# neeharperi/FutureDet

Hardware: AMD Instinct MI355X
Metric: sweeps/sec end-to-end (300k pts, 10-sweep voxel) (higher is better)
Workload: dtype f32

## Files before the change

### futuredet_amd/csrc/fd_spconv_c32.hip

```cpp
#include "fd_spconv_chunk.h"

namespace {

namespace sk = fd::skeleton;
typedef float f32x16 __attribute__((ext_vector_type(16)));
typedef unsigned u32x4 __attribute__((ext_vector_type(4)));
constexpr int TM = 128, COUT = 32, TS = 4, WR = 1;
constexpr sk::Layout L = sk::layout(TM, COUT, TS, 32);
static_assert(((sk::kMaxTaps + TS - 1) / TS) * (TM / WR / 32) <= L.item_slot, "item list slot");

template <int CIN, int DEPTH>
__global__ void __launch_bounds__(256) spconv_f32_c32(const float *__restrict__ in, const float4 *__restrict__ wp, const float *__restrict__ bias,
                                                      const float *__restrict__ residual, int relu, const int *__restrict__ nbr, int64_t nbr_stride,
                                                      int K, int n_out, const int *__restrict__ n_out_dev, float *__restrict__ out, unsigned in_bytes,
                                                      const int *__restrict__ ranges, int rows_per_range) {
    constexpr int NCH = CIN / 8;
    constexpr int kPad = sk::pad_entry(TM);
    extern __shared__ __attribute__((aligned(16))) unsigned char smem[];
    int *s_list = reinterpret_cast<int *>(smem + L.list);
    unsigned short *s_items = reinterpret_cast<unsigned short *>(smem + L.items);
    unsigned char *s_cnt = smem + L.cnt;
    int *s_pad = reinterpret_cast<int *>(smem + L.pad);
    float *s_acc = reinterpret_cast<float *>(smem + L.acc);

    const int tid = threadIdx.x, lane = tid & 63, wave = __builtin_amdgcn_readfirstlane(tid >> 6);
    int r_begin, r_end, n_chunks, chunk_rows;
    sk::resolve_range(n_out, n_out_dev, ranges, rows_per_range, r_begin, r_end);
    if (r_begin >= r_end) return;
    sk::cut_chunks<TM>(r_begin, r_end, n_chunks, chunk_rows);
    int pre[sk::kSliceRegs<TM>];
    sk::fetch_slice<TM>(pre, nbr, nbr_stride, K, r_begin);

    const int ln = lane & 31, lh = lane >> 5;
    const int ts = wave, wr = 0;
    unsigned char *acc_bytes = reinterpret_cast<unsigned char *>(s_acc + ts * L.acc_copy);
    const __amdgpu_buffer_rsrc_t rsrc = __builtin_amdgcn_make_buffer_rsrc(const_cast<float *>(in), 0, (int)in_bytes, 0x00020000);
    unsigned short *items = s_items + wave * L.item_slot;

    for (int chunk = 0; chunk < n_chunks; ++chunk) {
        int row0, n_rows;
        if (!sk::chunk_span(r_begin, r_end, chunk_rows, chunk, row0, n_rows)) break;
        sk::stage_chunk<TM, COUT, TS, 32>(pre, s_list, s_pad, s_acc, bias, residual, K, row0, n_rows);
        __syncthreads();
        sk::compact_taps<TM, WR>(s_list, s_cnt, K);
        __syncthreads();
        if (chunk + 1 < n_chunks) sk::fetch_slice<TM>(pre, nbr, nbr_stride, K, row0 + chunk_rows);
        const int n_items = sk::build_items<TS, 32>(s_cnt, items, K, ts, wr);

        int k_r[DEPTH], row_r[DEPTH];
        u32x4 a_r[DEPTH][NCH];
        auto stage_a0 = [&](int it) -> int { return sk::stage_a0(items, n_items, it); };
        auto stage_a1 = [&](int it, int code_v, int &kk, int &e) { sk::stage_a1<TM, WR, 32>(s_list, s_pad, n_items, wr, ln, it, code_v, kk, e); };
        auto gather_offset = [&](int e) -> unsigned { return sk::entry_row_bytes<CIN>(e) + (unsigned)(lh * 16); };
        auto gather_step = [&](unsigned voff, int c) { return __builtin_amdgcn_raw_buffer_load_b128(rsrc, voff + c * 32, 0, 0); };
        float4 b[NCH];
        auto load_b = [&](int k) {
            const float4 *wk = wp + (int64_t)k * NCH * 64 + lane;
#pragma unroll
            for (int c = 0; c < NCH; ++c) b[c] = wk[c * 64];
        };
        int k_s, e_s, code_s;
#pragma unroll
        for (int d = 0; d < DEPTH - 1; ++d) {
            stage_a1(d, stage_a0(d), k_s, e_s);
            const unsigned vo = gather_offset(e_s);
#pragma unroll
            for (int c = 0; c < NCH; ++c) a_r[d][c] = gather_step(vo, c);
            k_r[d] = k_s;
            row_r[d] = e_s;
        }
        k_r[DEPTH - 1] = -1;
        row_r[DEPTH - 1] = kPad;
        stage_a1(DEPTH - 1, stage_a0(DEPTH - 1), k_s, e_s);
        code_s = stage_a0(DEPTH);
        if (n_items > 0) load_b(k_r[0]);

        for (int i0 = 0; i0 < n_items; i0 += DEPTH) {
#pragma unroll
            for (int d = 0; d < DEPTH; ++d) {
                const unsigned arow = sk::entry_local_row(row_r[d]);
                unsigned aoff[4];
#pragma unroll
                for (int q = 0; q < 4; ++q) aoff[q] = sk::acc_slot_bytes<COUT>(arow, (unsigned)(2 * q + lh));
                f32x16 acc;
#pragma unroll
                for (int q = 0; q < 4; ++q) {
                    const float4 v = *reinterpret_cast<const float4 *>(acc_bytes + aoff[q]);
                    acc[4 * q + 0] = v.x; acc[4 * q + 1] = v.y; acc[4 * q + 2] = v.z; acc[4 * q + 3] = v.w;
                }
                const int dn = (d + DEPTH - 1) % DEPTH;
                {
                    const int it = i0 + d + DEPTH - 1;
                    const unsigned vo = gather_offset(e_s);
                    k_r[dn] = k_s;
                    row_r[dn] = e_s;
#pragma unroll
                    for (int c = 0; c < NCH; ++c) a_r[dn][c] = gather_step(vo, c);
                    stage_a1(it + 1, code_s, k_s, e_s);
                    code_s = stage_a0(it + 2);
                }
                const int knext = k_r[(d + 1) % DEPTH];
                const bool reload = knext >= 0 && knext != k_r[d];
                __builtin_amdgcn_sched_barrier(0);
#pragma unroll
                for (int c = 0; c < NCH; ++c) {
                    const float4 av = __builtin_bit_cast(float4, a_r[d][c]);
                    acc = __builtin_amdgcn_mfma_f32_32x32x2f32(b[c].x, av.x, acc, 0, 0, 0);
                    acc = __builtin_amdgcn_mfma_f32_32x32x2f32(b[c].y, av.y, acc, 0, 0, 0);
                    acc = __builtin_amdgcn_mfma_f32_32x32x2f32(b[c].z, av.z, acc, 0, 0, 0);
                    acc = __builtin_amdgcn_mfma_f32_32x32x2f32(b[c].w, av.w, acc, 0, 0, 0);
                    if (reload) b[c] = (wp + (int64_t)knext * NCH * 64 + lane)[c * 64];
                }
#pragma unroll
                for (int q = 0; q < 4; ++q)
                    *reinterpret_cast<float4 *>(acc_bytes + aoff[q]) = make_float4(acc[4 * q + 0], acc[4 * q + 1], acc[4 * q + 2], acc[4 * q + 3]);
                __builtin_amdgcn_sched_barrier(0);
            }
        }
        __syncthreads();
        sk::epilogue<TM, COUT, TS>(s_acc, bias, residual, relu, out, row0, n_rows);
        __syncthreads();
    }
}

template <int CIN, int DEPTH>
int launch_c32(const fd::SpconvCall &c) {
    const unsigned in_bytes = (unsigned)(c.n_in * CIN * 4);
    int n_ranges = c.n_ranges, rows_per = 0;
    if (!c.ranges) sk::equal_rows_split(c.n_out, TM, c.n_out_dev != nullptr, n_ranges, rows_per);
    static std::atomic<uint64_t> lds_set{0};
    if (!fd::ensure_dynamic_lds(reinterpret_cast<const void *>(spconv_f32_c32<CIN, DEPTH>), (size_t)L.bytes, lds_set)) return 0;
    const void *wp = (const char *)c.wpacked + fd::spconv_weight_layout(c).c32.offset;
    hipLaunchKernelGGL((spconv_f32_c32<CIN, DEPTH>), dim3((unsigned)n_ranges), dim3(256), (size_t)L.bytes, c.stream, (const float *)c.in, (const float4 *)wp,
                       c.bias, (const float *)c.residual, c.relu, c.nbr, c.nbr_stride, c.K, c.n_out, c.n_out_dev, (float *)c.out, in_bytes, c.ranges, rows_per);
    return 1;
}

}

namespace fd {
int spconv_f32_c32_dispatch(const SpconvCall &c) {
    if (c.cout != 32 || c.cin != 32) return 0;
    if (!sk::entries_fit(c.n_in, c.cin)) return 0;
    return launch_c32<32, 3>(c);
}
}
```

Measured before the change: 282.1.

## Keep per-wave tap weights resident in registers and cut pipeline depth

```diff
diff --git a/futuredet_amd/csrc/fd_spconv_c32.hip b/futuredet_amd/csrc/fd_spconv_c32.hip
--- a/futuredet_amd/csrc/fd_spconv_c32.hip
+++ b/futuredet_amd/csrc/fd_spconv_c32.hip
@@ -6,11 +6,12 @@
 typedef float f32x16 __attribute__((ext_vector_type(16)));
 typedef unsigned u32x4 __attribute__((ext_vector_type(4)));
 constexpr int TM = 128, COUT = 32, TS = 4, WR = 1;
+constexpr int NSET = (sk::kMaxTaps + TS - 1) / TS;
 constexpr sk::Layout L = sk::layout(TM, COUT, TS, 32);
 static_assert(((sk::kMaxTaps + TS - 1) / TS) * (TM / WR / 32) <= L.item_slot, "item list slot");
 
 template <int CIN, int DEPTH>
-__global__ void __launch_bounds__(256) spconv_f32_c32(const float *__restrict__ in, const float4 *__restrict__ wp, const float *__restrict__ bias,
+__global__ void __launch_bounds__(256) __attribute__((amdgpu_waves_per_eu(2, 2))) spconv_f32_c32(const float *__restrict__ in, const float4 *__restrict__ wp, const float *__restrict__ bias,
                                                       const float *__restrict__ residual, int relu, const int *__restrict__ nbr, int64_t nbr_stride,
                                                       int K, int n_out, const int *__restrict__ n_out_dev, float *__restrict__ out, unsigned in_bytes,
                                                       const int *__restrict__ ranges, int rows_per_range) {
@@ -28,11 +29,31 @@
     sk::resolve_range(n_out, n_out_dev, ranges, rows_per_range, r_begin, r_end);
     if (r_begin >= r_end) return;
     sk::cut_chunks<TM>(r_begin, r_end, n_chunks, chunk_rows);
-    int pre[sk::kSliceRegs<TM>];
-    sk::fetch_slice<TM>(pre, nbr, nbr_stride, K, r_begin);
-
     const int ln = lane & 31, lh = lane >> 5;
     const int ts = wave, wr = 0;
+    float4 w[NSET][NCH];
+#pragma unroll
+    for (int s = 0; s < NSET; ++s) {
+        const int k = ts + TS * s < K ? ts + TS * s : K - 1;
+        const float4 *wk = wp + (int64_t)k * NCH * 64 + lane;
+#pragma unroll
+        for (int c = 0; c < NCH; ++c) w[s][c] = wk[c * 64];
+    }
+    int pre[sk::kSliceRegs<TM>];
+    static_assert(256 % TM == 0 && 64 % (256 / TM) == 0, "a wave stays inside one tap");
+    auto fetch_slice = [&](int row0) {
+        int64_t o = (int64_t)row0 + tid % TM;
+        o = o < nbr_stride ? o : nbr_stride - 1;
+        const int *col = nbr + o;
+#pragma unroll
+        for (int i = 0; i < sk::kSliceRegs<TM>; ++i) {
+            int k = wave / (TM / 64) + i * (256 / TM);
+            k = k < K ? k : K - 1;
+            pre[i] = col[(int64_t)k * nbr_stride];
+        }
+    };
+    fetch_slice(r_begin);
+
     unsigned char *acc_bytes = reinterpret_cast<unsigned char *>(s_acc + ts * L.acc_copy);
     const __amdgpu_buffer_rsrc_t rsrc = __builtin_amdgcn_make_buffer_rsrc(const_cast<float *>(in), 0, (int)in_bytes, 0x00020000);
     unsigned short *items = s_items + wave * L.item_slot;
@@ -44,7 +65,7 @@
         __syncthreads();
         sk::compact_taps<TM, WR>(s_list, s_cnt, K);
         __syncthreads();
-        if (chunk + 1 < n_chunks) sk::fetch_slice<TM>(pre, nbr, nbr_stride, K, row0 + chunk_rows);
+        if (chunk + 1 < n_chunks) fetch_slice(row0 + chunk_rows);
         const int n_items = sk::build_items<TS, 32>(s_cnt, items, K, ts, wr);
 
         int k_r[DEPTH], row_r[DEPTH];
@@ -53,12 +74,6 @@
         auto stage_a1 = [&](int it, int code_v, int &kk, int &e) { sk::stage_a1<TM, WR, 32>(s_list, s_pad, n_items, wr, ln, it, code_v, kk, e); };
         auto gather_offset = [&](int e) -> unsigned { return sk::entry_row_bytes<CIN>(e) + (unsigned)(lh * 16); };
         auto gather_step = [&](unsigned voff, int c) { return __builtin_amdgcn_raw_buffer_load_b128(rsrc, voff + c * 32, 0, 0); };
-        float4 b[NCH];
-        auto load_b = [&](int k) {
-            const float4 *wk = wp + (int64_t)k * NCH * 64 + lane;
-#pragma unroll
-            for (int c = 0; c < NCH; ++c) b[c] = wk[c * 64];
-        };
         int k_s, e_s, code_s;
 #pragma unroll
         for (int d = 0; d < DEPTH - 1; ++d) {
@@ -68,12 +83,12 @@
             for (int c = 0; c < NCH; ++c) a_r[d][c] = gather_step(vo, c);
             k_r[d] = k_s;
             row_r[d] = e_s;
+            __builtin_amdgcn_sched_barrier(0);
         }
         k_r[DEPTH - 1] = -1;
         row_r[DEPTH - 1] = kPad;
         stage_a1(DEPTH - 1, stage_a0(DEPTH - 1), k_s, e_s);
         code_s = stage_a0(DEPTH);
-        if (n_items > 0) load_b(k_r[0]);
 
         for (int i0 = 0; i0 < n_items; i0 += DEPTH) {
 #pragma unroll
@@ -99,17 +114,20 @@
                     stage_a1(it + 1, code_s, k_s, e_s);
                     code_s = stage_a0(it + 2);
                 }
-                const int knext = k_r[(d + 1) % DEPTH];
-                const bool reload = knext >= 0 && knext != k_r[d];
                 __builtin_amdgcn_sched_barrier(0);
+                const int slot = k_r[d] >> 2;
+                static_assert(TS == 4 && NSET == 7, "tap -> weight set");
 #pragma unroll
-                for (int c = 0; c < NCH; ++c) {
-                    const float4 av = __builtin_bit_cast(float4, a_r[d][c]);
-                    acc = __builtin_amdgcn_mfma_f32_32x32x2f32(b[c].x, av.x, acc, 0, 0, 0);
-                    acc = __builtin_amdgcn_mfma_f32_32x32x2f32(b[c].y, av.y, acc, 0, 0, 0);
-                    acc = __builtin_amdgcn_mfma_f32_32x32x2f32(b[c].z, av.z, acc, 0, 0, 0);
-                    acc = __builtin_amdgcn_mfma_f32_32x32x2f32(b[c].w, av.w, acc, 0, 0, 0);
-                    if (reload) b[c] = (wp + (int64_t)knext * NCH * 64 + lane)[c * 64];
+                for (int s = 0; s < NSET; ++s) {
+                    if (slot != s) continue;
+#pragma unroll
+                    for (int c = 0; c < NCH; ++c) {
+                        const float4 av = __builtin_bit_cast(float4, a_r[d][c]);
+                        acc = __builtin_amdgcn_mfma_f32_32x32x2f32(w[s][c].x, av.x, acc, 0, 0, 0);
+                        acc = __builtin_amdgcn_mfma_f32_32x32x2f32(w[s][c].y, av.y, acc, 0, 0, 0);
+                        acc = __builtin_amdgcn_mfma_f32_32x32x2f32(w[s][c].z, av.z, acc, 0, 0, 0);
+                        acc = __builtin_amdgcn_mfma_f32_32x32x2f32(w[s][c].w, av.w, acc, 0, 0, 0);
+                    }
                 }
 #pragma unroll
                 for (int q = 0; q < 4; ++q)
@@ -142,6 +160,7 @@
 int spconv_f32_c32_dispatch(const SpconvCall &c) {
     if (c.cout != 32 || c.cin != 32) return 0;
     if (!sk::entries_fit(c.n_in, c.cin)) return 0;
-    return launch_c32<32, 3>(c);
+    if (fd::tuning(fd::kTuneSpconvC32) == 3) return launch_c32<32, 3>(c);
+    return launch_c32<32, 2>(c);
 }
 }
```

Result: no change. 282.3, median of 2 (+0.1%).
